# vitoplantamura/OnnxStream

Hardware: AMD Instinct MI355X
Metric: sd15_unet_step_latency_ms+images_per_sec_512x512_20step (higher is better)
Workload: dtype f16

## Files before the change

### onnxstream_amd/bindings.py

```python
import ctypes
import re
from typing import List

import numpy


class OnnxStreamError(Exception):
    pass


class _GetTensorReturnLayout(ctypes.Structure):
    _fields_ = [("dims_num", ctypes.c_size_t), ("dims", ctypes.c_void_p),
                ("data_num", ctypes.c_size_t), ("data", ctypes.c_void_p)]


_WP_NAMES = ("ram", "nocache", "prefetch", "ram+nocache", "ram+prefetch")


class Model:
    def __init__(self, library_path: str, threads_count: int = 0, weights_provider_name: str = "prefetch"):
        self._lib = ctypes.CDLL(library_path)
        self._proto()
        self.mangle_tensor_names = True
        if weights_provider_name not in _WP_NAMES:
# ... 216 lines not shown
                return bool(f(self._h, self._name(src), self._name(dst)))
        raise OnnxStreamError("this library cannot rename tensors through the C API")

    def hip_set_vram_budget(self, nbytes: int):
        f = self._lib.model_hip_set_vram_budget
        f.argtypes = [ctypes.c_void_p, ctypes.c_ulonglong]; f.restype = None
        f(self._h, int(nbytes))

    def hip_resident_weight_bytes(self) -> int:
        f = self._lib.model_hip_resident_weight_bytes
        f.argtypes = [ctypes.c_void_p]; f.restype = ctypes.c_ulonglong
        return int(f(self._h))

    def hip_read_range_data(self, filename: str):
        f = self._lib.model_hip_read_range_data
        f.argtypes = [ctypes.c_void_p, ctypes.c_char_p]; f.restype = ctypes.c_void_p
        self._err(f(self._h, filename.encode()))

    def hip_write_range_data(self, filename: str):
        f = self._lib.model_hip_write_range_data
        f.argtypes = [ctypes.c_void_p, ctypes.c_char_p]; f.restype = ctypes.c_void_p
        self._err(f(self._h, filename.encode()))

    def hip_plan_info(self) -> str:
        f = self._lib.model_hip_plan_info
        f.argtypes = [ctypes.c_void_p]; f.restype = ctypes.c_void_p
        p = f(self._h)
        text = ctypes.cast(p, ctypes.c_char_p).value.decode("utf-8", "replace")
        self._lib.model_free_buffer(p)
        if text.startswith("ERROR: "):
            raise OnnxStreamError(text[7:])
        return text

    def hip_profile(self, reps: int = 1):
        f = self._lib.model_hip_profile
        f.argtypes = [ctypes.c_void_p, ctypes.c_int]; f.restype = ctypes.c_void_p
        p = f(self._h, reps)
        text = ctypes.cast(p, ctypes.c_char_p).value.decode("utf-8", "replace")
        self._lib.model_free_buffer(p)
        if text.startswith("ERROR: "):
            raise OnnxStreamError(text[7:])
        rows = []
        for line in text.splitlines():
            ms, fl, by, what = line.split("\t", 3)
            rows.append((float(ms), float(fl), float(by), what))
        return rows

    def hip_last_pass_ms(self) -> float:
        f = self._lib.model_hip_last_pass_ms
        f.argtypes = [ctypes.c_void_p]; f.restype = ctypes.c_double
        return f(self._h)

    def hip_streamed_bytes(self) -> int:
        f = self._lib.model_hip_streamed_bytes
        f.argtypes = [ctypes.c_void_p]; f.restype = ctypes.c_ulonglong
        return int(f(self._h))

    def hip_plans_built(self) -> int:
        f = self._lib.model_hip_plans_built
        f.restype = ctypes.c_ulonglong
        f.argtypes = [ctypes.c_void_p]
        return int(f(self._h))

    def hip_last_kernel_count(self) -> int:
        f = self._lib.model_hip_last_kernel_count
        f.argtypes = [ctypes.c_void_p]; f.restype = ctypes.c_ulonglong
# ... 15 lines not shown
```

### onnxstream_amd/csrc/host/exports.cpp

```cpp
#include <cstdio>
#include <cstring>

#include "onnxstream.h"
#include "plan.h"

using namespace onnxstream;

namespace {

char* dup_cstr(const std::string& s) {
    char* p = (char*)std::malloc(s.size() + 1);
    std::memcpy(p, s.c_str(), s.size() + 1);
    return p;
}

struct Handle {
    explicit Handle(int threads) : model(threads) {}
    Model model;
    std::string definition;
    std::string provider;
};

const char* dtype_name(TensorDataType t) {
    switch (t) {
// ... 173 lines not shown
}

void model_clear_tensors(Handle* h) { h->model.m_data.clear(); }

void model_set_option(Handle* h, char* name, unsigned int value) {
    Model& m = h->model;
    const std::string n = name;
    const bool b = value != 0;
    if (n == "use_fp16_arithmetic") m.m_use_fp16_arithmetic = b;
    else if (n == "use_uint8_qdq") m.m_use_uint8_qdq = b;
    else if (n == "use_uint8_arithmetic") m.m_use_uint8_arithmetic = b;
    else if (n == "fuse_ops_in_attention") m.m_fuse_ops_in_attention = b;
    else if (n == "force_fp16_storage") m.m_force_fp16_storage = b;
    else if (n == "support_dynamic_shapes") m.m_support_dynamic_shapes = b;
    else if (n == "use_ops_cache") m.m_use_ops_cache = b;
    else if (n == "use_scaled_dp_attn_op") m.m_use_scaled_dp_attn_op = b;
    else if (n == "use_next_op_cache") m.m_use_next_op_cache = b;
    else if (n == "ops_printf") m.m_ops_printf = b;
    else if (n == "ops_times_printf") m.m_ops_times_printf = b;
    else if (n == "use_nchw_convs") m.m_use_nchw_convs = b;
    else if (n == "range_data_calibrate") m.m_range_data_calibrate = b;
    else if (n == "attention_fused_ops_parts") m.m_attention_fused_ops_parts = value;
    else if (n == "hip_device") m.m_hip_device = (int)value;
    else if (n == "hip_fusion_level") m.m_hip_fusion_level = (int)value;
    else if (n == "hip_use_graph") m.m_hip_use_graph = b;
    else if (n == "hip_autotune") m.m_hip_autotune = b;
    else if (n == "hip_fuse_ln_gemm") m.m_hip_fuse_ln_gemm = b;
    else if (n == "hip_concat_views") m.m_hip_concat_views = b;
    else if (n == "hip_fuse_tblock") m.m_hip_fuse_tblock = b;
    else if (n == "hip_gn_stats") m.m_hip_gn_stats = (int)value;
    else if (n == "hip_stream_weights") m.m_hip_stream_weights = b;
    else if (n == "hip_w8_resident") m.m_hip_w8_resident = b;
    else if (n == "hip_resident_outputs") m.m_hip_resident_outputs = b;
    else {
        const char* err = "model_set_option: 'name' not found.";
        printf("=== ERROR === %s\n", err);
        throw std::invalid_argument(err);
    }
}

void model_add_extra_output(Handle* h, char* name) { h->model.m_extra_outputs.emplace_back(name); }

void model_free_buffer(void* ptr) { std::free(ptr); }

double model_hip_last_pass_ms(Handle* h) { return h->model.hip_last_pass_ms(); }
unsigned long long model_hip_last_kernel_count(Handle* h) { return h->model.hip_last_kernel_count(); }
void model_hip_invalidate_plan(Handle* h) { h->model.hip_invalidate_plan(); }
unsigned long long model_hip_plans_built(Handle* h) { return h->model.hip_plans_built(); }
unsigned long long model_hip_streamed_bytes(Handle* h) { return h->model.hip_streamed_bytes(); }
unsigned long long model_hip_resident_weight_bytes(Handle* h) { return h->model.hip_resident_weight_bytes(); }
void model_hip_set_vram_budget(Handle* h, unsigned long long bytes) { h->model.set_cuda_options(CudaOptions(bytes, false)); }
void model_hip_set_upcast_substrings(Handle* h, const char* list) {
    std::vector<std::string> subs;
    std::string cur;
    for (const char* p = list ? list : ""; ; p++) {
        if (*p == '|' || *p == 0) {
            if (!cur.empty()) subs.push_back(cur);
            cur.clear();
            if (!*p) break;
        } else cur.push_back(*p);
    }
    if (subs.empty()) h->model.m_requires_upcast = nullptr;
    else
        h->model.m_requires_upcast = [subs](const std::string&, const std::string& name) {
            for (auto& s : subs)
                if (name.find(s) != std::string::npos) return true;
// ... 37 lines not shown
        return dup_cstr(e.what());
    }
}
char* model_hip_sampler_loop(Handle* h, char* sample_name, char* timestep_name, char* out_name, int steps, int prompts, float* x, const float* noise,
                             const float* c_in, const float* c_out, const float* t, const float* sigma, const float* d_sigma, const float* sigma_up, float guidance, const float* clip,
                             double* ms) {
    try {
        const double v = h->model.hip_sampler_loop(sample_name, timestep_name, out_name, steps, prompts, x, noise, c_in, c_out, t, sigma, d_sigma, sigma_up, guidance, clip);
        if (ms) *ms = v;
        return nullptr;
    } catch (const std::exception& e) {
        return dup_cstr(e.what());
    }
}
char* model_hip_sampler_loop_multistep(Handle* h, char* sample_name, char* timestep_name, char* out_name, int steps, int prompts, int sampler, float* x,
                                       const float* c_in, const float* c_out, const float* t, const float* sigma, const int* order, const float* coef,
                                       unsigned long long n_coef, const double* dcoef, unsigned long long n_dcoef, float guidance, double* ms) {
    try {
        const double v = Plan::run_sampler_loop_multistep(h->model, sample_name, timestep_name, out_name, steps, prompts, sampler, x, c_in, c_out, t,
                                                           sigma, order, coef, (size_t)n_coef, dcoef, (size_t)n_dcoef, guidance);
        if (ms) *ms = v;
        return nullptr;
    } catch (const std::exception& e) {
        return dup_cstr(e.what());
    }
}
char* model_hip_plan_info(Handle* h) {
    try {
        return dup_cstr(h->model.hip_plan_info());
    } catch (const std::exception& e) {
        return dup_cstr(std::string("ERROR: ") + e.what());
    }
}
char* model_hip_profile(Handle* h, int reps) {
    try {
        return dup_cstr(h->model.hip_profile(reps));
    } catch (const std::exception& e) {
        return dup_cstr(std::string("ERROR: ") + e.what());
    }
}

char* model_hip_read_range_data(Handle* h, const char* filename) {
    try {
        h->model.read_range_data(filename);
        return nullptr;
    } catch (const std::exception& e) {
        return dup_cstr(e.what());
    }
}
char* model_hip_write_range_data(Handle* h, const char* filename) {
    try {
        h->model.write_range_data(filename);
        return nullptr;
    } catch (const std::exception& e) {
        return dup_cstr(e.what());
    }
}

}
```

### onnxstream_amd/csrc/host/lowering_ops.inc

```
    void lower(const Operation& op) {
        const std::string& t = op.m_type;
        if (try_host_eval(op)) return;
        if (P.u8) return lower_u8(op);
        if (t == "Gather") return lower_gather(op);
        if (t == "Cast") return lower_cast(op);
        if (t == "Conv") {
            conv1d_out = Conv1dOut{};
            lower_conv(op);
            if (conv1d_out.y >= 0) {
                check_out(op, {1, conv1d_out.Cout, conv1d_out.Lo});
                P.alias(P.ensure_plain(conv1d_out.y), {1, conv1d_out.Cout, conv1d_out.Lo}, Lay::plain, op.m_output[0].m_name);
            }
            return;
        }
        if (t == "MatMul") return lower_matmul(op);
        if (t == "osg.Linear") return lower_linear(op);
        if (t == "Gemm") return lower_gemm(op);
        if (t == "Add" || t == "Sub" || t == "Mul" || t == "Div") return lower_binary(op);
        if (t == "Sigmoid" || t == "Erf" || t == "Sqrt" || t == "Sin" || t == "Cos" || t == "Neg" || t == "osg.SiLU") return lower_unary(op);
        if (t == "Pow") return lower_pow(op);
        if (t == "InstanceNormalization") return lower_instance_norm(op);
        if (t == "osg.GroupNorm") return lower_group_norm(op);
        if (t == "osg.LayerNorm") return lower_layer_norm(op);
        if (t == "osg.GEGLU") return lower_geglu(op);
// ... 714 lines not shown
            be.check(be.api.osg_instance_norm(be.ctx, OSG_F16, P.ptr(x), (const float*)P.ptr(sc), (const float*)P.ptr(bi), P.ptr(y), (int)rows, L,
                                              (int)G, eps),
                     "InstanceNormalization");
        });
    }

    void lower_group_norm(const Operation& op) {
        int x = P.ensure_nhwc(in_val(op.m_input[0]));
        int g = in_val(op.m_input[1]), b = in_val(op.m_input[2]);
        const Shape s = V(x).shape;
        const long G = std::stol(*attr(op, "groups"));
        const float eps = std::stof(*attr(op, "epsilon"));
        const int act = *attr(op, "silu") == "1" ? OSG_ACT_SILU : OSG_ACT_NONE;
        int y = out_val(op, s, Lay::nhwc, V(x).batched);
        const long nb = B(x), HW = s[2] * s[3], C = s[1];
        if (P.gn_stats_on && V(x).dtype == OSG_F16 && HW % 128 == 0 && nb * HW >= 2048 && nb * HW * C >= P.gn_stats_min_elems && C % 8 == 0 && C % G == 0 && V(x).ld == 0 && V(x).view_off == 0) {
            std::vector<ConcatPart> parts;
            const int rx = P.root_of(x);
            auto cp = concat_parts.find(rx);
            if (cp != concat_parts.end()) parts = cp->second;
            else {
                auto it = conv_producers.find(rx);
                if (it != conv_producers.end() && it->second.y == x && it->second.out->dst == x && it->second.out->dst_ld == 0) parts.push_back(ConcatPart{it->second.out, 0, 0, it->second.step});
            }
            bool ok = !parts.empty();
            for (auto& pt : parts) ok = ok && !pt.out->no_sinks && pt.out->sink[pt.slot].off < 0 && (pt.out->sink_hw == 0 || pt.out->sink_hw == (int)HW);
            if (ok) {
                const long off = P.gn_stats_bytes;
                P.gn_stats_bytes += (size_t)8 * nb * G * 2 * sizeof(long long);
                for (auto& pt : parts) {
                    pt.out->sink[pt.slot] = StatSinkRef{off, (int)G, (int)(C / G), (int)pt.ch_off};
                    pt.out->sink_hw = (int)HW;
                    P.steps[pt.step].what += " +gnstats";
                }
                P.add_step("GroupNorm stats< " + op.m_name, {x, g, b}, {y}, [=, this] {
                    be.check(be.api.osg_group_norm_stats_nhwc(be.ctx, P.ptr(x), P.ptr(g), P.ptr(b), P.ptr(y), (int)nb, HW, (int)C, (int)G, eps, (osg_act)act, P.gn_stats + off),
                             "GroupNorm");
                });
                return;
            }
        }
        P.add_step("GroupNorm " + op.m_name, {x, g, b}, {y}, [=, this] {
            be.check(be.api.osg_group_norm_nhwc(be.ctx, OSG_F16, P.ptr(x), P.ptr(g), P.ptr(b), P.ptr(y), (int)nb, HW, (int)C, (int)G, eps, (osg_act)act),
                     "GroupNorm");
        });
    }

    std::map<std::string, LnFold> ln_deferred;
    std::string ln_tag(const LnFold& f, int bias) {
        return "|ln:" + V(f.g).name + ":" + V(f.b).name + ":" + (bias >= 0 ? V(bias).name : std::string("-"));
    }

    bool ln_can_fold(const Operation& op, int x, int g, int b, long C) {
        if (P.fusion < 2 || !P.fuse_ln_gemm || P.stream_weights) return false;
        if (C % 64) return false;
        if (!V(g).host_valid || !V(b).host_valid || (long)V(g).host_f.size() != C || (long)V(b).host_f.size() != C) return false;
        if (V(x).ld != 0) return false;
        const std::string& out = op.m_output[0].m_name;
        if (use_count(out) >= 1000) return false;
        auto cit = consumers.find(out);
        if (cit == consumers.end() || cit->second.empty()) return false;
        int group = -2;
        for (int c : cit->second) {
            const Operation& co = ops()[c];
            if (dead[c] || co.m_type != "osg.Linear" || co.m_input.empty() || co.m_input[0].m_name != out) return false;
            for (size_t k = 1; k < co.m_input.size(); k++)
// ... 721 lines not shown
```

### onnxstream_amd/csrc/host/plan.cpp

```cpp
#include "plan.h"
#include "qu8.h"

#include <algorithm>
#include <chrono>
#include <cmath>
#include <cstdio>
#include <cstring>
#include <thread>
#include <string_view>
#include <unordered_map>
#include <unordered_set>

namespace onnxstream {

namespace {

using Shape = std::vector<long>;

long prod(const Shape& s, size_t from = 0, size_t to = (size_t)-1) {
    long n = 1;
    for (size_t i = from; i < std::min(to, s.size()); i++) n *= s[i];
    return n;
}

// ... 154 lines not shown
    for (int guard = 0; guard < 64; guard++) {
        if (vals[v].qsrc >= 0) v = vals[v].qsrc;
        else if (vals[v].root >= 0) v = vals[v].root;
        else break;
    }
    return vals[v];
}

void Plan::share_q(int dst, int src) {
    if (vals[src].dtype != OSG_U8 || dst == src) return;
    int s = src;
    while (vals[s].qsrc < 0 && vals[s].root >= 0) s = vals[s].root;
    if (vals[s].qsrc >= 0) s = vals[s].qsrc;
    int d = dst;
    while (vals[d].root >= 0) d = vals[d].root;
    if (d == s) return;
    vals[d].qsrc = s;
    vals[d].qscale = vals[s].qscale;
    vals[d].qzp = vals[s].qzp;
    vals[d].qdyn = vals[s].qdyn;
}

long Plan::total_elems(int v) const { return vals[v].numel() * (vals[v].batched ? N : 1); }
size_t Plan::val_bytes(int v) const { return (size_t)total_elems(v) * esize(vals[v].dtype); }

void* Plan::ptr(int v) const {
    size_t off = 0;
    while (vals[v].root >= 0) {
        off += vals[v].view_off;
        v = vals[v].root;
    }
    const Val& r = vals[v];
    if (r.dptr) return (char*)r.dptr + off;
    return (char*)arena + r.offset + off;
}

bool Plan::in_one_slab(const char* lo, const char* hi) const {
    for (auto& sl : slabs)
        if (lo >= sl.first && hi <= sl.first + sl.second) return true;
    return false;
}

void* Plan::small_alloc(size_t bytes) {
    const size_t need = (std::max<size_t>(bytes, 1) + 255) & ~(size_t)255;
    if (need > ((size_t)1 << 20)) {
        void* p = be.malloc(need);
        owned.push_back(p);
        return p;
    }
    if (need > slab_left) {
        slab_left = (size_t)8 << 20;
        slab = (char*)pooled_malloc(slab_left);
        slabs.push_back({slab, slab_left});
    }
    void* p = slab;
    slab += need;
    slab_left -= need;
    return p;
}

void* Plan::pooled_malloc(size_t bytes) {
    if (!recycle) {
        void* p = be.malloc(bytes);
        owned.push_back(p);
        return p;
    }
// ... 92 lines not shown
struct Lowering {
    Plan& P;
    Model& m;
    HipBackend& be;
    long N;
    std::unordered_map<std::string, int> uses;
    std::unordered_map<std::string, int> producer;
    std::unordered_map<std::string, std::vector<int>> consumers;
    std::vector<char> dead;
    std::map<std::string, int> const_cache;

    explicit Lowering(Plan& p) : P(p), m(p.m), be(p.be), N(p.N) {}

    std::vector<Operation>& ops() { return P.ops; }
    Val& V(int v) { return P.vals[v]; }
    osg_dtype act_dtype() const { return OSG_F16; }

#include "lowering_graph.inc"
#include "lowering_u8.inc"
#include "lowering_ops.inc"
};

Plan::~Plan() {
    if (in_flight) be.api.osg_sync(be.ctx);
    steps.clear();
    steps.shrink_to_fit();
    delete lowering;
    lowering = nullptr;
    for (auto& o : outputs)
        if (o.dev) pool.give_class(be, o.dev, ConstPool::size_class(o.dev_bytes));
    for (auto& r : recyclable) pool.give(be, r.first, r.second);
    for (auto& kv : registered) be.api.osg_host_unregister(be.ctx, (void*)kv.first);
    if (graph) be.api.osg_graph_destroy(graph);
    if (samp_x) be.api.osg_free(be.ctx, samp_x);
    if (samp_noise) be.api.osg_free(be.ctx, samp_noise);
    if (samp_hist) be.api.osg_free(be.ctx, samp_hist);
    if (ring) be.free(ring);
    for (void* p : owned) be.free(p);
    if (arena && !arena_pooled) be.free(arena);
}

void Plan::build() {
    if (!fp16 && !u8)
        throw std::runtime_error("Model::run: the HIP backend implements f16 arithmetic (m_use_fp16_arithmetic, the configuration the reference uses for "
                                 "the SD UNet, src/sd.cpp:1633) and uint8 arithmetic (m_use_uint8_arithmetic, src/sd.cpp:1218); fp32 arithmetic is not implemented.");
    if (m.m_use_uint8_qdq)
        throw std::runtime_error("Model::run: m_use_uint8_qdq (uint8 storage between fp32 ops) is not implemented on the HIP backend.");
    if (m.m_requires_upcast && u8)
        throw std::runtime_error("Model::run: m_requires_upcast with uint8 arithmetic is not implemented on the HIP backend.");
    if (calibrate) {
        if (u8) throw std::invalid_argument("Model::run: m_range_data_calibrate runs in floating-point arithmetic (src/sd.cpp:1216-1222), not with m_use_uint8_arithmetic.");
        fusion = 0;
    }
    if (calibrate && stream_weights)
        throw std::invalid_argument("Model::run: m_range_data_calibrate cannot be combined with streamed weights (hip_stream_weights / a VRAM budget) on the HIP backend: calibrate with resident weights.");
    if (u8) {
        if (N != 1) throw std::invalid_argument("Model::run: uint8 arithmetic runs one sample per pass on the HIP backend (every pushed sample is quantised with its own scale).");
        fusion = 0;
    }
    be.check(be.api.osg_set_autotune(be.ctx, m.m_hip_autotune ? 1 : 0), "osg_set_autotune");
    static const bool timing = std::getenv("OSG_PLAN_TIMING") != nullptr;
    auto now = [] { return std::chrono::steady_clock::now(); };
    auto ms_since = [&](std::chrono::steady_clock::time_point t0) { return std::chrono::duration<double, std::milli>(now() - t0).count(); };
    const auto t_begin = now();
    vals.reserve(m.m_ops.size() * 12 + 1024);
    lowering = new Lowering(*this);
// ... 276 lines not shown
```

### onnxstream_amd/csrc/host/plan.h

```cpp
#pragma once

#include <cmath>
#include <cstdint>
#include <functional>
#include <map>
#include <unordered_map>
#include <set>
#include <string>
#include <vector>

#include "backend.h"
#include "onnxstream.h"

namespace onnxstream {

enum class Lay { plain, nhwc };

struct Val {
    std::string name;
    std::vector<long> shape;
    osg_dtype dtype = OSG_F16;
    Lay lay = Lay::plain;
    bool batched = false;
    bool is_const = false;
    int root = -1;
    void* dptr = nullptr;
    size_t offset = 0;
    bool pinned = false;
    int first = 1 << 30, last = -1;
    std::vector<float> host_f;
    std::vector<int64_t> host_i;
    bool host_valid = false;
    bool up32 = false;
    bool host_only = false;
    int as_plain = -1, as_nhwc = -1, as_dense = -1;
    long ld = 0;
    size_t view_off = 0;
    float qscale = 1.f;
    int qzp = 0;
    int qsrc = -1;
    bool qdyn = false;
    int as_nk_u8 = -1;
    int rep_src = -1;
    long rep = 1;
    long numel() const { long n = 1; for (auto d : shape) n *= d; return n; }
};

struct Step {
    std::string what;
    std::function<void()> run;
    std::vector<int> reads, writes;
    double flops = 0;
};

struct Lowering;

struct ConstPool {
    struct Base {
        void* dptr = nullptr;
        size_t bytes = 0;
        std::vector<float> host_f;
        std::vector<int64_t> host_i;
        bool host_valid = false;
    };
    std::map<std::string, Base> base;
    std::map<std::string, std::pair<void*, size_t>> derived;
    std::vector<TensorDataType> occ_types;
    bool complete = false;
    size_t bytes = 0;
    std::string fused_key;
    std::vector<Operation> fused_ops;
    size_t fused_const_vals = 0;
    bool fused_valid = false;
    std::vector<Val> snap_vals;
    size_t snap_weight_bytes = 0;
    std::vector<std::string> in_names;
    std::vector<std::pair<void*, size_t>> spare;
    void* take(size_t bytes, size_t* got) {
        int best = -1;
        for (size_t i = 0; i < spare.size(); i++)
            if (spare[i].second >= bytes && (best < 0 || spare[i].second < spare[best].second)) best = (int)i;
        if (best < 0 || spare[best].second > 4 * bytes + ((size_t)8 << 20)) return nullptr;
        void* p = spare[best].first;
        *got = spare[best].second;
        spare.erase(spare.begin() + best);
        return p;
    }
    std::map<size_t, std::vector<void*>> spare_class;
    static size_t size_class(size_t bytes) {
        size_t c = 4096;
        while (c < bytes) c <<= 1;
        return c;
    }
    void* take_class(HipBackend& be, size_t cls) {
        auto it = spare_class.find(cls);
        if (it != spare_class.end() && !it->second.empty()) {
            void* p = it->second.back();
            it->second.pop_back();
            return p;
        }
        return be.malloc(cls);
    }
    void give_class(HipBackend& be, void* p, size_t cls) {
        auto& v = spare_class[cls];
        if (v.size() >= 512) be.free(p);
        else v.push_back(p);
    }
    void give(HipBackend& be, void* p, size_t bytes) {
        if (spare.size() >= 8) {
            size_t k = 0;
// ... 14 lines not shown
        spare_class.clear();
        base.clear(); derived.clear(); occ_types.clear();
        complete = false; bytes = 0;
        fused_valid = false; fused_ops.clear(); fused_key.clear(); snap_vals.clear(); snap_weight_bytes = 0; in_names.clear();
    }
};

inline float half_to_float(uint16_t h) {
    uint32_t sign = (h >> 15) & 1, exp = (h >> 10) & 0x1f, man = h & 0x3ff;
    float v;
    if (exp == 0) v = std::ldexp((float)man, -24);
    else if (exp == 31) v = man ? NAN : INFINITY;
    else v = std::ldexp((float)(man | 0x400), (int)exp - 25);
    return sign ? -v : v;
}

struct Plan {
    Plan(Model& m, HipBackend& be, ConstPool& pool, size_t batch);
    ~Plan();
    void build();
    void execute(const std::function<void()>& while_device_runs = nullptr);
    void replay(int n, float* ms_each);
    void set_input(const std::string& name, long index, const float* data, size_t count);
    double sampler_loop(const std::string& sample_name, const std::string& timestep_name, const std::string& out_name, int n_steps, int prompts,
                        float* x, const float* noise, const float* c_in, const float* c_out, const float* t, const float* sigma, const float* d_sigma,
                        const float* sigma_up, float guidance, const float* clip);
    double sampler_loop_multistep(const std::string& sample_name, const std::string& timestep_name, const std::string& out_name, int n_steps, int prompts,
                                  int sampler, float* x, const float* c_in, const float* c_out, const float* t, const float* sigma, const int* order,
                                  const float* coef, size_t n_coef, const double* dcoef, size_t n_dcoef, float guidance);
    static double run_sampler_loop_multistep(Model& m, const std::string& sample_name, const std::string& timestep_name, const std::string& out_name,
                                             int n_steps, int prompts, int sampler, float* x, const float* c_in, const float* c_out, const float* t,
                                             const float* sigma, const int* order, const float* coef, size_t n_coef, const double* dcoef, size_t n_dcoef,
                                             float guidance);
    std::string profile(int reps);
    std::string info() const;
    bool compatible(Model& m, size_t batch) const;
    size_t kernel_count() const { return steps.size(); }
    double last_ms() const { return m_last_ms; }

    Model& m;
    HipBackend& be;
    ConstPool& pool;
    long N;

    std::vector<Operation> ops;
    std::vector<Val> vals;
    std::unordered_map<std::string, int> by_name;
    std::vector<Step> steps;
    std::vector<char> io_block;
    size_t gathered_up = 0, gathered_down = 0;
    std::vector<std::pair<char*, size_t>> slabs;
    bool in_one_slab(const char* lo, const char* hi) const;
    std::vector<void*> owned;
    std::vector<std::pair<void*, size_t>> recyclable;
    bool recycle = false, arena_pooled = false;
    void* pooled_malloc(size_t bytes);
    void* small_alloc(size_t bytes);
    char* slab = nullptr;
    size_t slab_left = 0;
    void* arena = nullptr;
    size_t arena_bytes = 0, weight_bytes = 0;

    struct WRecipe {
        int val = -1;
        std::string fn;
        TensorDataType ty = TensorDataType::none;
// ... 28 lines not shown
        size_t dev_bytes = 0;
    };
    bool resident_outputs = false;
    struct Calib { int step; std::string op; int val; };
    std::vector<Calib> calib;
    std::vector<In> inputs;
    std::vector<Out> outputs;

    void* samp_x = nullptr;
    void* samp_noise = nullptr;
    void* samp_hist = nullptr;
    size_t samp_x_bytes = 0, samp_noise_bytes = 0, samp_hist_bytes = 0;

    osg_graph* graph = nullptr;
    Lowering* lowering = nullptr;
    int runs = 0;
    bool in_capture = false;
    double m_last_ms = 0;
    bool fp16 = true;
    bool u8_qdq = false, autotune = false, calibrate = false, fuse_attn = false, sdp_attn = false;
    std::set<std::string> outputs_convert_set;
    bool u8 = false;
    bool stream_weights = false;
    bool fuse_ln_gemm = false;
    bool concat_views = true;
    bool fuse_tblock = true;
    bool in_flight = false;
    bool gn_stats_on = false;
    int gn_stats_req = 2;
    long gn_stats_min_elems = 0;
    char* gn_stats = nullptr;
    size_t gn_stats_bytes = 0;
    void zero_gn_stats();
    void run_steps(size_t begin = 0, size_t end = (size_t)-1);
    size_t dyn_end = 0;
    bool w8_resident = false;
    int fusion = 2;
    int fusion_req = 2;
    std::vector<std::string> extra_outputs;

    int new_val(const std::string& name, const std::vector<long>& shape, osg_dtype dt, Lay lay, bool batched);
    int alias(int v, const std::vector<long>& shape, Lay lay, const std::string& name = "");
    int root_of(int v) const;
    void* ptr(int v) const;
    size_t val_bytes(int v) const;
    long total_elems(int v) const;
    void add_step(const std::string& what, std::vector<int> reads, std::vector<int> writes, std::function<void()> fn);
    const Val& qv(int v) const;
    void share_q(int dst, int src);
    int ensure_plain(int v);
    int ensure_nhwc(int v);
    void* const_alloc(const std::string& tag, size_t bytes, bool* fresh);
    int ensure_dense(int v);
};

}
```

### onnxstream_amd/csrc/host/plan_run.cpp

```cpp
#include "plan.h"
#include "qu8.h"

#include <algorithm>
#include <chrono>
#include <cmath>
#include <cstdio>
#include <cstring>
#include <thread>
#include <string_view>
#include <unordered_map>
#include <unordered_set>

namespace onnxstream {

void Plan::zero_gn_stats() {
    if (gn_stats_bytes) be.check(be.api.osg_memset(be.ctx, gn_stats, 0, gn_stats_bytes), "osg_memset");
}

void Plan::run_steps(size_t begin, size_t end) {
    static const std::vector<std::string> skip = [] {
        std::vector<std::string> v;
        if (const char* e = std::getenv("OSG_PLAN_SKIP")) {
            std::string t = e;
            size_t b0 = 0;
            while (b0 <= t.size()) {
                size_t e0 = t.find(',', b0);
                if (e0 == std::string::npos) e0 = t.size();
                if (e0 > b0) v.push_back(t.substr(b0, e0 - b0));
                b0 = e0 + 1;
            }
        }
        return v;
    }();
    end = std::min(end, steps.size());
    if (begin == 0) zero_gn_stats();
    for (size_t si_ = begin; si_ < end; si_++) {
        Step& s = steps[si_];
        if (!skip.empty()) {
            bool sk = false;
            for (auto& pre : skip) sk |= s.what.rfind(pre, 0) == 0;
            if (sk) continue;
        }
        static const bool roctx_on = std::getenv("OSG_ROCTX") != nullptr;
        struct Range {
            HipBackend& b; bool on;
            Range(HipBackend& b_, bool on_, const char* n) : b(b_), on(on_) { if (on) b.api.osg_range_push(n); }
            ~Range() { if (on) b.api.osg_range_pop(); }
        } range(be, roctx_on, s.what.c_str());
        s.run();
        static const int extra_trivial = std::getenv("OSG_PROBE_EXTRA_TRIVIAL") ? atoi(std::getenv("OSG_PROBE_EXTRA_TRIVIAL")) : 0;
        if (extra_trivial > 0) {
            static void* probe = nullptr;
            if (!probe) be.check(be.api.osg_malloc(be.ctx, 4096, &probe), "osg_malloc");
            for (int k = 0; k < extra_trivial; k++)
                be.check(be.api.osg_convert(be.ctx, OSG_F32, OSG_F16, probe, (char*)probe + 2048, 4, 1.0f, 0), "osg_convert");
        }
        static const bool trace = std::getenv("OSG_PLAN_TRACE") != nullptr;
        if (trace && !in_capture) {
            fprintf(stderr, "[step] %s\n", s.what.c_str());
            be.check(be.api.osg_sync(be.ctx), "osg_sync");
        }
    }
}

void Plan::execute(const std::function<void()>& while_device_runs) {
    {
        bool moved = false;
        for (auto& o : outputs)
            if (o.dev_bytes && !o.dev) {
                o.dev = pool.take_class(be, ConstPool::size_class(o.dev_bytes));
                vals[o.f32val].dptr = o.dev;
                moved = true;
            }
        if (moved && graph) {
            be.api.osg_graph_destroy(graph);
            graph = nullptr;
        }
    }
    static const bool exec_times = getenv("OSG_EXEC_TIMES") != nullptr;
    const auto t_exec = std::chrono::steady_clock::now();
    auto ms_since = [](std::chrono::steady_clock::time_point t0) { return std::chrono::duration<double, std::milli>(std::chrono::steady_clock::now() - t0).count(); };
    double ms_stage = 0, ms_enqueue = 0, ms_wait = 0;
    char* up_lo = nullptr;
    char* up_hi = nullptr;
    {
        size_t sum = 0, cnt = 0;
        for (auto& in : inputs) {
            if (in.host_type != TensorDataType::float16 || vals[in.staging].numel() == 0 || in.resident) continue;
            char* p = (char*)ptr(in.val);
            const size_t nb = val_bytes(in.val);
            if (!up_lo || p < up_lo) up_lo = p;
            if (!up_hi || p + nb > up_hi) up_hi = p + nb;
            sum += (nb + 255) & ~(size_t)255;
            cnt++;
        }
        if (cnt < 4 || (size_t)(up_hi - up_lo) > sum || !in_one_slab(up_lo, up_hi)) up_lo = up_hi = nullptr;
        else io_block.assign((size_t)(up_hi - up_lo), 0);
    }
    for (auto& in : inputs) {
        Tensor* src = nullptr;
        for (auto& t : m.m_data)
            if (t.m_name == in.name) { src = &t; break; }
        if (!src) throw std::invalid_argument("Model::get_tensor_data: input tensor not found: " + in.name);
        if (src->m_type != in.host_type || src->m_shape != in.shape)
            throw std::invalid_argument("Model::run: input '" + in.name + "' changed type or shape since the plan was built.");
        if (in.host_type == TensorDataType::int64 || vals[in.staging].numel() == 0) continue;
        if (in.resident) {
            if (src->m_hip_resident != in.resident) throw std::invalid_argument("Model::run: input '" + in.name + "' changed since the plan was built.");
            continue;
        }
        if (in.host_type == TensorDataType::float16) {
            if (src->m_hip_resident) throw std::invalid_argument("Model::run: input '" + in.name + "' changed since the plan was built.");
            auto& vec = src->get_vector<uint16_t>();
            if (vec.size() != (size_t)vals[in.val].numel()) throw std::invalid_argument("Model::get_tensor_data: mismatch between tensor shape and data size.");
            if (up_lo) std::memcpy(io_block.data() + ((char*)ptr(in.val) - up_lo), vec.data(), vec.size() * 2);
// ... 286 lines not shown
    explicit FlightGuard(bool& f_) : f(f_) { f = true; }
    ~FlightGuard() { if (!std::uncaught_exceptions()) f = false; }
};
}

void Plan::replay(int n, float* ms_each) {
    if (!graph) throw std::runtime_error("Model::hip_replay: no captured pass yet (run() at least twice with hip_use_graph on).");
    FlightGuard flight(in_flight);
    if (!ms_each) {
        be.check(be.api.osg_timer_start(be.ctx), "osg_timer_start");
        for (int i = 0; i < n; i++) be.check(be.api.osg_graph_launch(be.ctx, graph), "osg_graph_launch");
        float ms = 0;
        be.check(be.api.osg_timer_stop(be.ctx, &ms), "osg_timer_stop");
        m_last_ms = n > 0 ? ms / n : 0;
        return;
    }
    for (int i = 0; i < n; i++) {
        be.check(be.api.osg_timer_start(be.ctx), "osg_timer_start");
        be.check(be.api.osg_graph_launch(be.ctx, graph), "osg_graph_launch");
        float ms = 0;
        be.check(be.api.osg_timer_stop(be.ctx, &ms), "osg_timer_stop");
        ms_each[i] = ms;
        m_last_ms = ms;
    }
}

void Plan::set_input(const std::string& name, long index, const float* data, size_t count) {
    if (u8) throw std::runtime_error("Model::hip_set_input: not available with uint8 arithmetic (inputs are quantised per run).");
    for (auto& in : inputs)
        if (in.name == name) {
            const size_t per = (size_t)vals[in.staging].numel();
            if (count != per) throw std::invalid_argument("Model::get_tensor_data: mismatch between tensor shape and data size.");
            if (index < 0 || index >= N) throw std::invalid_argument("Model::hip_set_input: sample index out of range.");
            be.check(be.api.osg_upload(be.ctx, (char*)ptr(in.staging) + index * per * sizeof(float), data, per * sizeof(float)), "osg_upload");
            return;
        }
    throw std::invalid_argument("Model::get_tensor_data: input tensor not found: " + name);
}

double Plan::sampler_loop(const std::string& sample_name, const std::string& timestep_name, const std::string& out_name, int n_steps, int prompts,
                          float* x, const float* noise, const float* c_in, const float* c_out, const float* t, const float* sigma, const float* d_sigma,
                          const float* sigma_up, float guidance, const float* clip) {
    if (runs < 1) throw std::runtime_error("Model::hip_sampler_loop: run() once first (the context inputs must be resident).");
    if (stream_weights) throw std::runtime_error("Model::hip_sampler_loop: not available in streamed-weights mode.");
    if (u8) throw std::runtime_error("Model::hip_sampler_loop: not available with uint8 arithmetic.");
    if (prompts <= 0 || 2L * prompts != N) throw std::invalid_argument("Model::hip_sampler_loop: the plan's batch must be 2 * prompts (cond, uncond per prompt).");
    FlightGuard flight(in_flight);
    const In *in_s = nullptr, *in_t = nullptr;
    for (auto& in : inputs) {
        if (in.name == sample_name) in_s = &in;
        if (in.name == timestep_name) in_t = &in;
    }
    const Out* out = nullptr;
    for (auto& o : outputs)
        if (o.name == out_name) out = &o;
    if (!in_s || !in_t || !out) throw std::invalid_argument("Model::hip_sampler_loop: input/output tensor not found.");
    if (out->raw16) throw std::invalid_argument("Model::hip_sampler_loop: the output is excluded from the fp32 conversion (m_outputs_convert_set).");
    const long L = vals[in_s->staging].numel(), TL = vals[in_t->staging].numel();
    if (vals[out->f32val].numel() != L || !vals[out->f32val].batched)
        throw std::invalid_argument("Model::hip_sampler_loop: the output must have the shape of the sample input.");
    const size_t xb = (size_t)prompts * L * sizeof(float), nb = (size_t)n_steps * xb;
    auto grow = [&](void*& p, size_t& have, size_t need) {
        if (have >= need) return;
        if (p) be.check(be.api.osg_free(be.ctx, p), "osg_free");
        p = nullptr;
        have = 0;
        be.check(be.api.osg_malloc(be.ctx, need, &p), "osg_malloc");
        have = need;
    };
    grow(samp_x, samp_x_bytes, xb);
    if (noise) grow(samp_noise, samp_noise_bytes, nb);
    be.check(be.api.osg_upload(be.ctx, samp_x, x, xb), "osg_upload");
    if (noise) be.check(be.api.osg_upload(be.ctx, samp_noise, noise, nb), "osg_upload");
    be.check(be.api.osg_timer_start(be.ctx), "osg_timer_start");
    for (int i = 0; i < n_steps; i++) {
        be.check(be.api.osg_sampler_prepare(be.ctx, (const float*)samp_x, (float*)ptr(in_s->staging), (float*)ptr(in_t->staging), prompts, L, c_in[i], t[i], TL),
                 "osg_sampler_prepare");
        if (graph) be.check(be.api.osg_graph_launch(be.ctx, graph), "osg_graph_launch");
        else run_steps();
        const bool with_noise = noise != nullptr;
        be.check(be.api.osg_sampler_cfg_euler_a(be.ctx, (float*)samp_x, (const float*)ptr(out->f32val),
                                               with_noise ? (const float*)samp_noise + (size_t)i * prompts * L : nullptr, prompts, L, c_out[i], guidance,
                                               sigma[i], d_sigma[i], sigma_up[i], clip ? clip[i] : 0.f),
                 "osg_sampler_cfg_euler_a");
    }
    float ms = 0;
    be.check(be.api.osg_timer_stop(be.ctx, &ms), "osg_timer_stop");
    be.check(be.api.osg_download(be.ctx, x, samp_x, xb), "osg_download");
    runs += n_steps;
    m_last_ms = n_steps > 0 ? ms / n_steps : 0;
    return ms;
}

double Plan::sampler_loop_multistep(const std::string& sample_name, const std::string& timestep_name, const std::string& out_name, int n_steps,
                                   int prompts, int sampler, float* x, const float* c_in, const float* c_out, const float* t, const float* sigma,
                                   const int* order, const float* coef, size_t n_coef, const double* dcoef, size_t n_dcoef, float guidance) {
    static const char* fn = "Model::hip_sampler_loop_multistep: ";
    if (runs < 1) throw std::runtime_error(std::string(fn) + "run() once first (the context inputs must be resident).");
    if (stream_weights) throw std::runtime_error(std::string(fn) + "not available in streamed-weights mode.");
    if (u8) throw std::runtime_error(std::string(fn) + "not available with uint8 arithmetic.");
    if (prompts <= 0 || 2L * prompts != N) throw std::invalid_argument(std::string(fn) + "the plan's batch must be 2 * prompts (cond, uncond per prompt).");
    static const int forms[6][4] = {
        {OSG_MS_DPMPP_FIRST, OSG_MS_DPMPP_2M, -1, -1},
        {OSG_MS_EULER_D, OSG_MS_IPNDM1, OSG_MS_IPNDM2, OSG_MS_IPNDM3},
        {OSG_MS_EULER_D, OSG_MS_IPNDM_V1, OSG_MS_IPNDM2, OSG_MS_IPNDM3},
        {OSG_MS_EULER_D, OSG_MS_IPNDM_VO1, OSG_MS_IPNDM_VO2, OSG_MS_IPNDM_VO3},
        {OSG_MS_EULER_D, OSG_MS_TAYLOR1, OSG_MS_TAYLOR2, -1},
        {OSG_MS_DDIM, -1, -1, -1},
    };
    static const int depth[6] = {1, 4, 4, 4, 3, 0};
    if (sampler < 0 || sampler >= 6) throw std::invalid_argument(std::string(fn) + "unknown sampler form " + std::to_string(sampler) + ".");
    if (n_steps < 0 || n_coef != (size_t)n_steps * 6 || n_dcoef != (size_t)n_steps * 2)
        throw std::invalid_argument(std::string(fn) + "the coefficient tables must hold steps * 6 floats and steps * 2 doubles.");
    for (int i = 0; i < n_steps; i++)
        if (order[i] < 0 || order[i] > 3 || order[i] > i || forms[sampler][order[i]] < 0)
            throw std::invalid_argument(std::string(fn) + "order " + std::to_string(order[i]) + " at step " + std::to_string(i) + " is not available.");
    FlightGuard flight(in_flight);
    const In *in_s = nullptr, *in_t = nullptr;
    for (auto& in : inputs) {
        if (in.name == sample_name) in_s = &in;
        if (in.name == timestep_name) in_t = &in;
    }
    const Out* out = nullptr;
    for (auto& o : outputs)
        if (o.name == out_name) out = &o;
    if (!in_s || !in_t || !out) throw std::invalid_argument(std::string(fn) + "input/output tensor not found.");
    if (out->raw16) throw std::invalid_argument(std::string(fn) + "the output is excluded from the fp32 conversion (m_outputs_convert_set).");
    const long L = vals[in_s->staging].numel(), TL = vals[in_t->staging].numel();
    if (vals[out->f32val].numel() != L || !vals[out->f32val].batched)
        throw std::invalid_argument(std::string(fn) + "the output must have the shape of the sample input.");
    const int H = depth[sampler];
    const size_t xb = (size_t)prompts * L * sizeof(float), hb = (size_t)H * xb;
    auto grow = [&](void*& p, size_t& have, size_t need) {
        if (have >= need) return;
        if (p) be.check(be.api.osg_free(be.ctx, p), "osg_free");
        p = nullptr;
        have = 0;
        be.check(be.api.osg_malloc(be.ctx, need, &p), "osg_malloc");
        have = need;
    };
    grow(samp_x, samp_x_bytes, xb);
    if (H) grow(samp_hist, samp_hist_bytes, hb);
    be.check(be.api.osg_upload(be.ctx, samp_x, x, xb), "osg_upload");
    auto slot = [&](int i, int k) -> float* { return H ? (float*)samp_hist + (size_t)(((i - k) % H + H) % H) * prompts * L : nullptr; };
    be.check(be.api.osg_timer_start(be.ctx), "osg_timer_start");
    for (int i = 0; i < n_steps; i++) {
        const float* k = coef + (size_t)i * 6;
        if (sampler == 5)
            be.check(be.api.osg_sampler_prepare_rescale(be.ctx, (float*)samp_x, (float*)ptr(in_s->staging), (float*)ptr(in_t->staging), prompts, L, k[5],
                                                        c_in[i], t[i], TL),
                     "osg_sampler_prepare_rescale");
        else
            be.check(be.api.osg_sampler_prepare(be.ctx, (const float*)samp_x, (float*)ptr(in_s->staging), (float*)ptr(in_t->staging), prompts, L, c_in[i],
                                                t[i], TL),
                     "osg_sampler_prepare");
        if (graph) be.check(be.api.osg_graph_launch(be.ctx, graph), "osg_graph_launch");
        else run_steps();
        const int o = order[i];
        be.check(be.api.osg_sampler_cfg_multistep(be.ctx, forms[sampler][o], (float*)samp_x, (const float*)ptr(out->f32val), slot(i, 0),
                                                  o >= 1 ? slot(i, 1) : nullptr, o >= 2 ? slot(i, 2) : nullptr, o >= 3 ? slot(i, 3) : nullptr, prompts, L,
                                                  c_out[i], guidance, sigma[i], k[0], k[1], k[2], k[3], k[4], dcoef[2 * i], dcoef[2 * i + 1]),
                 "osg_sampler_cfg_multistep");
    }
    float ms = 0;
    be.check(be.api.osg_timer_stop(be.ctx, &ms), "osg_timer_stop");
    be.check(be.api.osg_download(be.ctx, x, samp_x, xb), "osg_download");
    runs += n_steps;
    m_last_ms = n_steps > 0 ? ms / n_steps : 0;
    return ms;
}

double Plan::run_sampler_loop_multistep(Model& m, const std::string& sample_name, const std::string& timestep_name, const std::string& out_name,
                                       int n_steps, int prompts, int sampler, float* x, const float* c_in, const float* c_out, const float* t,
                                       const float* sigma, const int* order, const float* coef, size_t n_coef, const double* dcoef, size_t n_dcoef,
                                       float guidance) {
    if (!m.m_plan) throw std::runtime_error("Model::hip_sampler_loop_multistep: no plan (call run() first).");
    const double ms = m.m_plan->sampler_loop_multistep(sample_name, timestep_name, out_name, n_steps, prompts, sampler, x, c_in, c_out, t, sigma, order,
                                                       coef, n_coef, dcoef, n_dcoef, guidance);
    m.m_last_ms = m.m_plan->last_ms();
    return ms;
}

std::string Plan::info() const {
    std::string out;
    char buf[128];
    for (size_t i = 0; i < steps.size(); i++) {
        const Step& s = steps[i];
        snprintf(buf, sizeof buf, "step %zu reads=", i);
        out += buf;
// ... 58 lines not shown
```

Measured before the change: 10.11.

## Hoist loop-invariant UNet steps out of the sampler loop graph

```diff
diff --git a/onnxstream_amd/bindings.py b/onnxstream_amd/bindings.py
--- a/onnxstream_amd/bindings.py
+++ b/onnxstream_amd/bindings.py
@@ -272,6 +272,16 @@
             raise OnnxStreamError(text[7:])
         return text
 
+    def hip_loop_info(self, sample: str, timestep: str) -> str:
+        f = self._lib.model_hip_loop_info
+        f.argtypes = [ctypes.c_void_p, ctypes.c_char_p, ctypes.c_char_p]; f.restype = ctypes.c_void_p
+        p = f(self._h, self._name(sample), self._name(timestep))
+        text = ctypes.cast(p, ctypes.c_char_p).value.decode("utf-8", "replace")
+        self._lib.model_free_buffer(p)
+        if text.startswith("ERROR: "):
+            raise OnnxStreamError(text[7:])
+        return text
+
     def hip_profile(self, reps: int = 1):
         f = self._lib.model_hip_profile
         f.argtypes = [ctypes.c_void_p, ctypes.c_int]; f.restype = ctypes.c_void_p
diff --git a/onnxstream_amd/csrc/host/exports.cpp b/onnxstream_amd/csrc/host/exports.cpp
--- a/onnxstream_amd/csrc/host/exports.cpp
+++ b/onnxstream_amd/csrc/host/exports.cpp
@@ -229,6 +229,7 @@
     else if (n == "hip_stream_weights") m.m_hip_stream_weights = b;
     else if (n == "hip_w8_resident") m.m_hip_w8_resident = b;
     else if (n == "hip_resident_outputs") m.m_hip_resident_outputs = b;
+    else if (n == "hip_loop_hoist") Plan::set_loop_hoist(m, b);
     else {
         const char* err = "model_set_option: 'name' not found.";
         printf("=== ERROR === %s\n", err);
@@ -332,6 +333,13 @@
         return dup_cstr(std::string("ERROR: ") + e.what());
     }
 }
+char* model_hip_loop_info(Handle* h, char* sample_name, char* timestep_name) {
+    try {
+        return dup_cstr(Plan::loop_info(h->model, sample_name, timestep_name));
+    } catch (const std::exception& e) {
+        return dup_cstr(std::string("ERROR: ") + e.what());
+    }
+}
 char* model_hip_profile(Handle* h, int reps) {
     try {
         return dup_cstr(h->model.hip_profile(reps));
diff --git a/onnxstream_amd/csrc/host/lowering_ops.inc b/onnxstream_amd/csrc/host/lowering_ops.inc
--- a/onnxstream_amd/csrc/host/lowering_ops.inc
+++ b/onnxstream_amd/csrc/host/lowering_ops.inc
@@ -770,6 +770,7 @@
                     pt.out->sink[pt.slot] = StatSinkRef{off, (int)G, (int)(C / G), (int)pt.ch_off};
                     pt.out->sink_hw = (int)HW;
                     P.steps[pt.step].what += " +gnstats";
+                    P.steps[pt.step].side_writes = true;
                 }
                 P.add_step("GroupNorm stats< " + op.m_name, {x, g, b}, {y}, [=, this] {
                     be.check(be.api.osg_group_norm_stats_nhwc(be.ctx, P.ptr(x), P.ptr(g), P.ptr(b), P.ptr(y), (int)nb, HW, (int)C, (int)G, eps, (osg_act)act, P.gn_stats + off),
diff --git a/onnxstream_amd/csrc/host/plan.cpp b/onnxstream_amd/csrc/host/plan.cpp
--- a/onnxstream_amd/csrc/host/plan.cpp
+++ b/onnxstream_amd/csrc/host/plan.cpp
@@ -210,6 +210,7 @@
     }
     const Val& r = vals[v];
     if (r.dptr) return (char*)r.dptr + off;
+    if (loop_addr && r.loop_ptr) return (char*)r.loop_ptr + off;
     return (char*)arena + r.offset + off;
 }
 
@@ -368,6 +369,7 @@
     for (auto& r : recyclable) pool.give(be, r.first, r.second);
     for (auto& kv : registered) be.api.osg_host_unregister(be.ctx, (void*)kv.first);
     if (graph) be.api.osg_graph_destroy(graph);
+    drop_loop_form();
     if (samp_x) be.api.osg_free(be.ctx, samp_x);
     if (samp_noise) be.api.osg_free(be.ctx, samp_noise);
     if (samp_hist) be.api.osg_free(be.ctx, samp_hist);
diff --git a/onnxstream_amd/csrc/host/plan.h b/onnxstream_amd/csrc/host/plan.h
--- a/onnxstream_amd/csrc/host/plan.h
+++ b/onnxstream_amd/csrc/host/plan.h
@@ -25,6 +25,7 @@
     bool is_const = false;
     int root = -1;
     void* dptr = nullptr;
+    void* loop_ptr = nullptr;
     size_t offset = 0;
     bool pinned = false;
     int first = 1 << 30, last = -1;
@@ -51,6 +52,7 @@
     std::function<void()> run;
     std::vector<int> reads, writes;
     double flops = 0;
+    bool side_writes = false;
 };
 
 struct Lowering;
@@ -76,6 +78,7 @@
     size_t snap_weight_bytes = 0;
     std::vector<std::string> in_names;
     std::vector<std::pair<void*, size_t>> spare;
+    bool loop_hoist = true;
     void* take(size_t bytes, size_t* got) {
         int best = -1;
         for (size_t i = 0; i < spare.size(); i++)
@@ -156,6 +159,24 @@
                                              int n_steps, int prompts, int sampler, float* x, const float* c_in, const float* c_out, const float* t,
                                              const float* sigma, const int* order, const float* coef, size_t n_coef, const double* dcoef, size_t n_dcoef,
                                              float guidance);
+    struct LoopForm {
+        bool marked = false;
+        std::string sample, timestep;
+        std::vector<char> invariant;
+        size_t n_invariant = 0;
+        std::vector<int> kept;
+        std::vector<void*> bufs;
+        osg_graph* graph = nullptr;
+        bool valid = false;
+    };
+    LoopForm loop;
+    bool loop_addr = false;
+    void mark_loop_invariant(const std::string& sample_name, const std::string& timestep_name);
+    osg_graph* loop_pass(const std::string& sample_name, const std::string& timestep_name);
+    void refresh_loop_pass(osg_graph* g);
+    void drop_loop_form();
+    static std::string loop_info(Model& m, const std::string& sample_name, const std::string& timestep_name);
+    static void set_loop_hoist(Model& m, bool on);
     std::string profile(int reps);
     std::string info() const;
     bool compatible(Model& m, size_t batch) const;
@@ -250,7 +271,7 @@
     char* gn_stats = nullptr;
     size_t gn_stats_bytes = 0;
     void zero_gn_stats();
-    void run_steps(size_t begin = 0, size_t end = (size_t)-1);
+    void run_steps(size_t begin = 0, size_t end = (size_t)-1, int part = -1);
     size_t dyn_end = 0;
     bool w8_resident = false;
     int fusion = 2;
diff --git a/onnxstream_amd/csrc/host/plan_run.cpp b/onnxstream_amd/csrc/host/plan_run.cpp
--- a/onnxstream_amd/csrc/host/plan_run.cpp
+++ b/onnxstream_amd/csrc/host/plan_run.cpp
@@ -17,7 +17,7 @@
     if (gn_stats_bytes) be.check(be.api.osg_memset(be.ctx, gn_stats, 0, gn_stats_bytes), "osg_memset");
 }
 
-void Plan::run_steps(size_t begin, size_t end) {
+void Plan::run_steps(size_t begin, size_t end, int part) {
     static const std::vector<std::string> skip = [] {
         std::vector<std::string> v;
         if (const char* e = std::getenv("OSG_PLAN_SKIP")) {
@@ -33,9 +33,10 @@
         return v;
     }();
     end = std::min(end, steps.size());
-    if (begin == 0) zero_gn_stats();
+    if (begin == 0 && part != 1) zero_gn_stats();
     for (size_t si_ = begin; si_ < end; si_++) {
         Step& s = steps[si_];
+        if (part >= 0 && (loop.invariant[si_] != 0) != (part == 1)) continue;
         if (!skip.empty()) {
             bool sk = false;
             for (auto& pre : skip) sk |= s.what.rfind(pre, 0) == 0;
@@ -75,12 +76,14 @@
         if (moved && graph) {
             be.api.osg_graph_destroy(graph);
             graph = nullptr;
+            drop_loop_form();
         }
     }
     static const bool exec_times = getenv("OSG_EXEC_TIMES") != nullptr;
     const auto t_exec = std::chrono::steady_clock::now();
     auto ms_since = [](std::chrono::steady_clock::time_point t0) { return std::chrono::duration<double, std::milli>(std::chrono::steady_clock::now() - t0).count(); };
     double ms_stage = 0, ms_enqueue = 0, ms_wait = 0;
+    loop.valid = false;
     char* up_lo = nullptr;
     char* up_hi = nullptr;
     {
@@ -433,10 +436,135 @@
             const size_t per = (size_t)vals[in.staging].numel();
             if (count != per) throw std::invalid_argument("Model::get_tensor_data: mismatch between tensor shape and data size.");
             if (index < 0 || index >= N) throw std::invalid_argument("Model::hip_set_input: sample index out of range.");
+            if (!loop.marked || (name != loop.sample && name != loop.timestep)) loop.valid = false;
             be.check(be.api.osg_upload(be.ctx, (char*)ptr(in.staging) + index * per * sizeof(float), data, per * sizeof(float)), "osg_upload");
             return;
         }
     throw std::invalid_argument("Model::get_tensor_data: input tensor not found: " + name);
+}
+
+void Plan::mark_loop_invariant(const std::string& sample_name, const std::string& timestep_name) {
+    loop.marked = true;
+    loop.sample = sample_name;
+    loop.timestep = timestep_name;
+    loop.invariant.assign(steps.size(), 1);
+    loop.kept.clear();
+    std::vector<char> variant(vals.size(), 0);
+    for (auto& in : inputs)
+        if (in.name == sample_name || in.name == timestep_name) variant[root_of(in.staging)] = variant[root_of(in.val)] = 1;
+    for (size_t si = 0; si < steps.size(); si++)
+        if (steps[si].side_writes || si < dyn_end) loop.invariant[si] = 0;
+    for (bool changed = true; changed;) {
+        changed = false;
+        for (size_t si = 0; si < steps.size(); si++) {
+            const Step& s = steps[si];
+            bool var = !loop.invariant[si];
+            bool spread = false;
+            if (!var) {
+                for (int v : s.reads) var |= variant[root_of(v)] != 0;
+                for (int v : s.writes) var |= variant[root_of(v)] != 0;
+            }
+            if (var)
+                for (int v : s.writes)
+                    if (!variant[root_of(v)]) variant[root_of(v)] = 1, spread = true;
+            if (var && loop.invariant[si]) loop.invariant[si] = 0, changed = true;
+            changed |= spread;
+        }
+    }
+    loop.n_invariant = 0;
+    std::set<int> kept;
+    for (size_t si = 0; si < steps.size(); si++) {
+        if (!loop.invariant[si]) continue;
+        loop.n_invariant++;
+        for (int v : steps[si].writes) {
+            const Val& r = vals[root_of(v)];
+            if (!r.dptr && !r.is_const && r.last >= 0) kept.insert(root_of(v));
+        }
+    }
+    loop.kept.assign(kept.begin(), kept.end());
+}
+
+void Plan::drop_loop_form() {
+    if (loop.graph) be.api.osg_graph_destroy(loop.graph);
+    for (void* p : loop.bufs) be.api.osg_free(be.ctx, p);
+    for (int v : loop.kept) vals[v].loop_ptr = nullptr;
+    loop = LoopForm();
+}
+
+osg_graph* Plan::loop_pass(const std::string& sample_name, const std::string& timestep_name) {
+    if (!graph || !pool.loop_hoist || dyn_end) return graph;
+    if (!loop.marked || loop.sample != sample_name || loop.timestep != timestep_name) {
+        drop_loop_form();
+        mark_loop_invariant(sample_name, timestep_name);
+    }
+    if (!loop.n_invariant) return graph;
+    if (loop.graph) return loop.graph;
+    for (size_t k = loop.bufs.size(); k < loop.kept.size(); k++) {
+        const int v = loop.kept[k];
+        void* p = nullptr;
+        be.check(be.api.osg_malloc(be.ctx, std::max<size_t>(val_bytes(v), 256), &p), "osg_malloc");
+        loop.bufs.push_back(p);
+        vals[v].loop_ptr = p;
+    }
+    loop.valid = false;
+    struct Addr {
+        bool& f;
+        explicit Addr(bool& f_) : f(f_) { f = true; }
+        ~Addr() { f = false; }
+    } addr(loop_addr);
+    be.check(be.api.osg_graph_begin(be.ctx), "osg_graph_begin");
+    in_capture = true;
+    try {
+        run_steps(0, (size_t)-1, 0);
+        in_capture = false;
+    } catch (...) {
+        in_capture = false;
+        osg_graph* g = nullptr;
+        be.api.osg_graph_end(be.ctx, &g);
+        if (g) be.api.osg_graph_destroy(g);
+        throw;
+    }
+    be.check(be.api.osg_graph_end(be.ctx, &loop.graph), "osg_graph_end");
+    return loop.graph;
+}
+
+void Plan::refresh_loop_pass(osg_graph* g) {
+    if (!g || g != loop.graph || loop.valid) return;
+    loop_addr = true;
+    try {
+        run_steps(0, (size_t)-1, 1);
+    } catch (...) {
+        loop_addr = false;
+        throw;
+    }
+    loop_addr = false;
+    loop.valid = true;
+}
+
+std::string Plan::loop_info(Model& m, const std::string& sample_name, const std::string& timestep_name) {
+    if (!m.m_plan) throw std::runtime_error("Model::hip_loop_info: no plan (call run() first).");
+    Plan& p = *m.m_plan;
+    bool have_s = false, have_t = false;
+    for (auto& in : p.inputs) {
+        have_s |= in.name == sample_name;
+        have_t |= in.name == timestep_name;
+    }
+    if (!have_s || !have_t) throw std::invalid_argument("Model::hip_loop_info: input tensor not found.");
+    if (!p.loop.marked || p.loop.sample != sample_name || p.loop.timestep != timestep_name) {
+        p.drop_loop_form();
+        p.mark_loop_invariant(sample_name, timestep_name);
+    }
+    std::string out;
+    for (size_t si = 0; si < p.steps.size(); si++)
+        if (p.loop.invariant[si]) out += "invariant " + std::to_string(si) + "\n";
+    for (int v : p.loop.kept) out += "kept " + std::to_string(v) + " bytes=" + std::to_string(p.val_bytes(v)) + "\n";
+    out += "loop_steps " + std::to_string(p.steps.size() - p.loop.n_invariant) + "\n";
+    return out;
+}
+
+void Plan::set_loop_hoist(Model& m, bool on) {
+    if (!m.m_pool) m.m_pool = new ConstPool();
+    m.m_pool->loop_hoist = on;
 }
 
 double Plan::sampler_loop(const std::string& sample_name, const std::string& timestep_name, const std::string& out_name, int n_steps, int prompts,
@@ -473,11 +601,13 @@
     if (noise) grow(samp_noise, samp_noise_bytes, nb);
     be.check(be.api.osg_upload(be.ctx, samp_x, x, xb), "osg_upload");
     if (noise) be.check(be.api.osg_upload(be.ctx, samp_noise, noise, nb), "osg_upload");
+    osg_graph* const pass = loop_pass(sample_name, timestep_name);
     be.check(be.api.osg_timer_start(be.ctx), "osg_timer_start");
+    refresh_loop_pass(pass);
     for (int i = 0; i < n_steps; i++) {
         be.check(be.api.osg_sampler_prepare(be.ctx, (const float*)samp_x, (float*)ptr(in_s->staging), (float*)ptr(in_t->staging), prompts, L, c_in[i], t[i], TL),
                  "osg_sampler_prepare");
-        if (graph) be.check(be.api.osg_graph_launch(be.ctx, graph), "osg_graph_launch");
+        if (pass) be.check(be.api.osg_graph_launch(be.ctx, pass), "osg_graph_launch");
         else run_steps();
         const bool with_noise = noise != nullptr;
         be.check(be.api.osg_sampler_cfg_euler_a(be.ctx, (float*)samp_x, (const float*)ptr(out->f32val),
@@ -544,7 +674,9 @@
     if (H) grow(samp_hist, samp_hist_bytes, hb);
     be.check(be.api.osg_upload(be.ctx, samp_x, x, xb), "osg_upload");
     auto slot = [&](int i, int k) -> float* { return H ? (float*)samp_hist + (size_t)(((i - k) % H + H) % H) * prompts * L : nullptr; };
+    osg_graph* const pass = loop_pass(sample_name, timestep_name);
     be.check(be.api.osg_timer_start(be.ctx), "osg_timer_start");
+    refresh_loop_pass(pass);
     for (int i = 0; i < n_steps; i++) {
         const float* k = coef + (size_t)i * 6;
         if (sampler == 5)
@@ -555,7 +687,7 @@
             be.check(be.api.osg_sampler_prepare(be.ctx, (const float*)samp_x, (float*)ptr(in_s->staging), (float*)ptr(in_t->staging), prompts, L, c_in[i],
                                                 t[i], TL),
                      "osg_sampler_prepare");
-        if (graph) be.check(be.api.osg_graph_launch(be.ctx, graph), "osg_graph_launch");
+        if (pass) be.check(be.api.osg_graph_launch(be.ctx, pass), "osg_graph_launch");
         else run_steps();
         const int o = order[i];
         be.check(be.api.osg_sampler_cfg_multistep(be.ctx, forms[sampler][o], (float*)samp_x, (const float*)ptr(out->f32val), slot(i, 0),
```

Result: no change. 10.10 (-0.1%).
